# jkulhanek/wild-gaussians

Measured on AMD Instinct MI355X. Metric: train_iters_per_s (fwd+bwd of the rasterizer, 1M Gaussians @1080p), higher is better.
Workload: dtype f32

## Files before the change

wild-gaussians_amd/build.py:

```python
#!/usr/bin/env python3
from __future__ import annotations

import os
import subprocess
import sys
from concurrent.futures import ThreadPoolExecutor

HERE = os.path.dirname(os.path.abspath(__file__))
CSRC = os.path.join(HERE, "csrc")
OBJ = os.path.join(HERE, "build")
OUT = os.path.join(HERE, "diff_gaussian_rasterization", "libwg_rasterizer.so")
INCLUDE = os.path.join(os.path.dirname(HERE), "include")

VARIANT = os.environ.get("WG_BUILD_VARIANT", "")
EXTRA = os.environ.get("WG_EXTRA_FLAGS", "").split()
FILE_EXTRA = {k: v.split() for k, v in (kv.split(":", 1) for kv in filter(None, os.environ.get("WG_FILE_FLAGS", "").split(";")))}
if VARIANT:
    OBJ = os.path.join(OBJ, VARIANT)
    OUT = os.path.join(OBJ, "libwg_rasterizer.so")
HIPCC = os.environ.get("HIPCC", "/opt/rocm/bin/hipcc")
COMMON = ["--offload-arch=gfx950", "-O3", "-std=c++17", "-fPIC", "-Wall", "-Wno-unused-function", "-I" + INCLUDE, "-I" + CSRC]
SOURCES = {
    "preprocess.hip": ["-ffp-contract=off", "-fno-slp-vectorize"],
    "project/project.hip": ["-ffp-contract=off", "-fno-slp-vectorize"],
# ... 5 lines not shown
    "binning.hip": ["-fno-slp-vectorize"],
    "render_fwd.hip": ["-fno-slp-vectorize"],
    "render_bwd.hip": ["-munsafe-fp-atomics", "-fno-slp-vectorize"],
    "colour_bwd/fixed_order.hip": ["-fno-slp-vectorize"],
    "preprocess_bwd.hip": ["-fno-slp-vectorize"],
    "api.hip": [],
    "knn.hip": ["-ffp-contract=off"],
    "ssim.hip": [],
    "activations.hip": ["-ffp-contract=off"],
    "densify.hip": [],
    "sh_eval.hip": [],
    "adam.hip": ["-ffp-contract=off"],
    "adam/adam_rows.hip": ["-ffp-contract=off"],
    "appearance/mlp.hip": [],
    "appearance/colour.hip": [],
    "appearance/rows.hip": [],
    "uncertainty/uncertainty.hip": [],
    "frames/frames.hip": [],
    "metrics/metrics.hip": ["-ffp-contract=off"],
    "dino/vit.hip": [],
    "lpips/lpips.hip": ["-ffp-contract=off"],
    "loss/step_loss.hip": [],
}
HEADERS = ["wg_common.h", "wg_alpha.h", "wg_sort.h", "wg_act.h", os.path.join("distortion", "distortion.h"), os.path.join(INCLUDE, "wg_rasterizer.h"), os.path.join(INCLUDE, "wg_knn.h"),
           os.path.join(INCLUDE, "wg_ssim.h"), os.path.join(INCLUDE, "wg_activations.h"), os.path.join(INCLUDE, "wg_densify.h"), os.path.join(INCLUDE, "wg_adam.h"), os.path.join(INCLUDE, "wg_adam_rows.h"), os.path.join(INCLUDE, "wg_sh_eval.h"),
           os.path.join(INCLUDE, "wg_filter3d.h"), os.path.join(INCLUDE, "wg_densify_prune.h"), os.path.join(INCLUDE, "wg_msssim.h"),
           os.path.join(INCLUDE, "wg_appearance_mlp.h"), os.path.join(INCLUDE, "wg_appearance_colour.h"),
           os.path.join(INCLUDE, "wg_appearance_rows.h"),
           os.path.join(INCLUDE, "wg_uncertainty.h"), os.path.join(INCLUDE, "wg_frames.h"),
           os.path.join(INCLUDE, "wg_metrics.h"), os.path.join(INCLUDE, "wg_dino.h"), os.path.join(INCLUDE, "wg_lpips.h"),
           os.path.join(INCLUDE, "wg_step_loss.h")]


def _newer(target: str, deps) -> bool:
    if not os.path.exists(target):
        return True
    t = os.path.getmtime(target)
    return any(os.path.getmtime(d) > t for d in deps)


def build(force: bool = False, verbose: bool = False) -> str:
    os.makedirs(OBJ, exist_ok=True)
    hdrs = [h if os.path.isabs(h) else os.path.join(CSRC, h) for h in HEADERS] + [os.path.abspath(__file__)]
    jobs = []
    objs = []
    for src, extra in SOURCES.items():
        s = os.path.join(CSRC, src)
# ... 92 lines not shown
```

wild-gaussians_amd/csrc/api.hip:

```cpp
#include "wg_common.h"
#include "distortion/distortion.h"

#include <dlfcn.h>
#include <limits>

#include <algorithm>
#include <atomic>
#include <chrono>
#include <cstdio>
#include <cstdlib>
#include <cstring>
#include <map>
#include <mutex>
#include <string>
#include <vector>

namespace {

thread_local std::string g_last_hip_error;

int hip_fail(hipError_t e, const char* where) {
    g_last_hip_error = std::string(where) + ": " + hipGetErrorString(e);
    return WG_ERR_HIP;
}
// ... 510 lines not shown
        g_order_tables.push_back({dev, nullptr, 0});
        return nullptr;
    }
    g_order_tables.push_back({dev, static_cast<uint32_t*>(p), slots});
    *slots_out = slots;
    return static_cast<uint32_t*>(p);
}
void order_tables_release() {
    std::lock_guard<std::mutex> l(g_order_mu);
    for (OrderTable& t : g_order_tables)
        if (t.mem) {
            int cur = 0;
            const bool sw = hipGetDevice(&cur) == hipSuccess && cur != t.dev && hipSetDevice(t.dev) == hipSuccess;
            (void)hipFree(t.mem);
            if (sw) (void)hipSetDevice(cur);
        }
    g_order_tables.clear();
}

struct FrameMode { const void* image; int exact; int row; const void* geom; size_t clean_floats; };
std::atomic<uint64_t> g_row_frames{0}, g_row_backwards{0};
std::atomic<uint64_t> g_clean_frames{0}, g_clean_backwards{0};
std::atomic<uint64_t> g_sh_skip_backwards{0};
std::atomic<uint64_t> g_contribution_calls{0};
std::atomic<uint64_t> g_depth_grad_backwards{0};
std::atomic<uint64_t> g_distortion_calls{0}, g_distortion_grad_backwards{0};
std::mutex g_mode_mu;
FrameMode g_modes[64];
unsigned g_mode_head = 0;
const void* image_key(const char* image_buffer) {
    return reinterpret_cast<const void*>((reinterpret_cast<uintptr_t>(image_buffer) + wg::ALIGN - 1) & ~(uintptr_t)(wg::ALIGN - 1));
}
void remember_mode(const char* image_buffer, int exact, int row, const char* geom_buffer, size_t clean_floats) {
    const void* k = image_key(image_buffer);
    const void* gk = image_key(geom_buffer);
    std::lock_guard<std::mutex> l(g_mode_mu);
    for (auto& m : g_modes)
        if (m.image == k) { m.exact = exact; m.row = row; m.geom = gk; m.clean_floats = clean_floats; return; }
    g_modes[g_mode_head++ % 64] = {k, exact, row, gk, clean_floats};
}
bool take_record_clean(const char* image_buffer, const char* geom_buffer, size_t floats) {
    const void* k = image_key(image_buffer);
    const void* gk = image_key(geom_buffer);
    std::lock_guard<std::mutex> l(g_mode_mu);
    for (auto& m : g_modes)
        if (m.image == k) {
// ... 522 lines not shown
#endif
        if (e != hipSuccess) return hip_fail(e, "deterministic backward scratch");
    }
    const size_t record_floats = (size_t)P * (wg::GRAD_REC_FLOATS + (dual ? 1 : 0));
    bool record_clean = take_record_clean(a.image_buffer, a.geom_buffer, record_floats) && record && !det && R > 0;
    if (record_clean) {
        hipStreamCaptureStatus capturing = hipStreamCaptureStatusNone;
        if (hipStreamIsCapturing(stream, &capturing) != hipSuccess) { (void)hipGetLastError(); record_clean = false; }
        else if (capturing != hipStreamCaptureStatusNone) record_clean = false;
    }
    if (record_clean) g_clean_backwards.fetch_add(1, std::memory_order_relaxed);
    const bool clear_records = record && !det && !record_clean;
    if (clear_records && R <= 0) {
        StageScope scope_(WG_STAGE_RENDER_BACKWARD, stream);
        hipError_t e = hipMemsetAsync(geom.grad_rec, 0, (size_t)P * (wg::GRAD_REC_FLOATS + (dual ? 1 : 0)) * sizeof(float), stream);
        if (e != hipSuccess) return hip_fail(e, "gradient record memset");
    }
    const bool sh_fill = WG_SH_GRAD_SKIP != 0 && R > 0 && shs != nullptr && dL_dsh != nullptr && tone == nullptr && tone2 == nullptr && !sh_second && !dual;
    const bool nt_stream = opt.sh_stream == 1 || (opt.sh_stream < 0 && P <= opt.sh_stream_max_p);
    if (sh_fill) g_sh_skip_backwards.fetch_add(1, std::memory_order_relaxed);
    if (R > 0) {
        float* const clear_ptr = det ? reinterpret_cast<float*>(det_flags) : (clear_records ? geom.grad_rec : nullptr);
        const size_t clear_floats = det ? ((size_t)R + 3) / 4 : (size_t)P * (wg::GRAD_REC_FLOATS + (dual ? 1 : 0));
        WG_STAGE(WG_STAGE_TILE_RANGES, wg::launch_tile_order(img.tile_last, nullptr, img.order_bwd, gx * gy, clear_ptr, clear_floats, opt.backward_order_period, stream), "tile_order");
        WG_STAGE(WG_STAGE_RENDER_BACKWARD, wg::launch_render_backward(width, height, gx, gy, img, bin, geom, subpixel_offset, background, dL_dpix,
                                            dL_dmean2D, dL_dconic, dL_dopacity, dL_dcolor, record, opt.exact_compositing != 0, dual ? second->dL_dpix2 : nullptr, det_slots, det_flags, (size_t)R, P, stream,
                                            sh_fill ? dL_dsh : nullptr, sh_fill ? (size_t)P * (size_t)M * 3 : 0, WG_SH_GRAD_FILL_NT != 0 && nt_stream),
                 "render_backward");
    }
    if (dgrad != nullptr) {
        {
            StageScope scope_(WG_STAGE_RENDER_DEPTH_BACKWARD, stream);
            hipError_t e = hipMemsetAsync(dgrad->dL_dvalues, 0, (size_t)P * sizeof(float), stream);
            if (e != hipSuccess) return hip_fail(e, "dL_dvalues memset");
        }
        if (R > 0) {
            g_depth_grad_backwards.fetch_add(1, std::memory_order_relaxed);
            WG_STAGE(WG_STAGE_RENDER_DEPTH_BACKWARD, wg::launch_render_depth_backward(width, height, gx, gy, img, bin, geom, subpixel_offset, dgrad->dL_ddepth,
                                                                                    dgrad->values, means3D, campos, dgrad->dL_dvalues,
                                                                                    opt.exact_compositing != 0, stream), "render_depth_backward");
        }
    }
    if (tgrad != nullptr) {
        {
            StageScope scope_(WG_STAGE_RENDER_DEPTH_BACKWARD, stream);
            hipError_t e = hipMemsetAsync(tgrad->dL_dvalues, 0, (size_t)P * sizeof(float), stream);
            if (e != hipSuccess) return hip_fail(e, "distortion dL_dvalues memset");
        }
        if (R > 0) {
            g_distortion_grad_backwards.fetch_add(1, std::memory_order_relaxed);
// ... 301 lines not shown
    out->order_key = img.order_key;
    out->order_bwd = img.order_bwd;
    return WG_OK;
}

enum class OptKind { Flag, Tri, Range, ClampLow, ZeroOneOr };
struct OptionRow {
    const char* name;
    int (*get)(const wg::Options&);
    void (*set)(wg::Options&, int);
    OptKind kind; int lo, hi;
    void (*after_set)();
};
#define WG_OPTION(name, member, ...) {name, [](const wg::Options& o) { return (int)o.member; }, [](wg::Options& o, int v) { o.member = static_cast<decltype(o.member)>(v); }, __VA_ARGS__}
static const OptionRow g_option_rows[] = {
    WG_OPTION("force_global_sort", force_global_sort, OptKind::Flag, 0, 0, nullptr),
    WG_OPTION("host_mailbox", use_mailbox, OptKind::Flag, 0, 0, nullptr),
    WG_OPTION("geometry_reuse", geometry_reuse, OptKind::Flag, 0, 0, nullptr),
    WG_OPTION("fused_scan", fused_scan, OptKind::Flag, 0, 0, nullptr),
    WG_OPTION("forward_order", forward_order, OptKind::Flag, 0, 0, nullptr),
    WG_OPTION("forward_order_slots", forward_order_slots, OptKind::Range, 0, 1 << 16, nullptr),
    WG_OPTION("order_period", order_period, OptKind::Range, 0, 4096, nullptr),
    WG_OPTION("backward_order_period", backward_order_period, OptKind::Range, 0, 4096, nullptr),
    WG_OPTION("lazy_colour", lazy_colour, OptKind::Flag, 0, 0, nullptr),
    WG_OPTION("lazy_colour_min_p", lazy_colour_min_p, OptKind::Range, 0, 0x7fffffff, nullptr),
    WG_OPTION("sh_stream", sh_stream, OptKind::Tri, 0, 0, nullptr),
    WG_OPTION("sh_stream_max_p", sh_stream_max_p, OptKind::Range, 0, 0x7fffffff, nullptr),
    WG_OPTION("speculative_forward", speculative, OptKind::Range, 0, 2, [] { t_spec.clear(); t_wait.clear(); t_deferred.pending = false; }),
    WG_OPTION("spec_margin_pct", spec_margin_pct, OptKind::Range, 0, 1000, nullptr),
    WG_OPTION("band_list_min_p", band_list_min_p, OptKind::ClampLow, 1, 0, nullptr),
    WG_OPTION("near_split", near_split, OptKind::Tri, 0, 0, [] { t_split.reset(true); }),
    WG_OPTION("near_per_tile", near_per_tile, OptKind::ClampLow, 0, 0, nullptr),
    WG_OPTION("near_adapt", near_adapt, OptKind::Flag, 0, 0, [] { t_split.reset(false); }),
    WG_OPTION("box_count", box_count, OptKind::Tri, 0, 0, nullptr),
    WG_OPTION("depth_codes", depth_codes, OptKind::ZeroOneOr, 8, 12, nullptr),
    WG_OPTION("staged_scatter", staged_scatter, OptKind::Tri, 0, 0, nullptr),
    WG_OPTION("staged_scatter_cap", staged_cap, OptKind::ClampLow, 0, 0, nullptr),
    WG_OPTION("lazy_sort", lazy.enabled, OptKind::Flag, 0, 0, nullptr),
    WG_OPTION("lazy_min_len", lazy.min_len, OptKind::Range, 256, 2048, nullptr),
    WG_OPTION("lazy_target", lazy.target, OptKind::Range, 1, 2048, nullptr),
    WG_OPTION("lazy_cap", lazy.cap, OptKind::Range, 1, 2048, nullptr),
};
#undef WG_OPTION
static const OptionRow* find_option(const char* name) {
    for (const OptionRow& r : g_option_rows)
        if (std::strcmp(name, r.name) == 0) return &r;
// ... 25 lines not shown
    r->set(g_opt, value);
    if (r->after_set) r->after_set();
    return WG_OK;
}

int wg_get_option(const char* name) {
    if (!name) return -1;
    if (std::strcmp(name, "roctx") == 0) return g_roctx.enabled ? 1 : 0;
    if (std::strcmp(name, "near_split_backoff") == 0) return (int)t_split.backoff;
    if (std::strcmp(name, "near_per_tile_now") == 0) return (int)t_split.near.cur;
    if (std::strcmp(name, "near_floor_now") == 0) return (int)t_split.near.floor;
    if (std::strcmp(name, "near_far_tiles_last") == 0) return (int)t_split.near.last_far;
    if (std::strcmp(name, "spec_frames") == 0) return (int)std::min<uint64_t>(t_wait.spec_frames, 0x7fffffffu);
    if (std::strcmp(name, "spec_misses") == 0) return (int)std::min<uint64_t>(t_wait.spec_misses, 0x7fffffffu);
    if (std::strcmp(name, "forward_polls") == 0) return (int)std::min<uint64_t>(t_wait.polls, 0x7fffffffu);
    if (std::strcmp(name, "forward_polls_waited") == 0) return (int)std::min<uint64_t>(t_wait.waited, 0x7fffffffu);
    if (std::strcmp(name, "forward_wait_us_total") == 0) return (int)std::min(t_wait.wait_us, 2147483647.0);
    if (std::strcmp(name, "forward_wait_us_last") == 0) return (int)std::min(t_wait.last_wait_us, 2147483647.0);
    if (std::strcmp(name, "backward_row_frames") == 0) return (int)std::min<uint64_t>(g_row_frames.load(std::memory_order_relaxed), 0x7fffffffu);
    if (std::strcmp(name, "backward_row_calls") == 0) return (int)std::min<uint64_t>(g_row_backwards.load(std::memory_order_relaxed), 0x7fffffffu);
    if (std::strcmp(name, "record_clean_frames") == 0) return (int)std::min<uint64_t>(g_clean_frames.load(std::memory_order_relaxed), 0x7fffffffu);
    if (std::strcmp(name, "record_clean_calls") == 0) return (int)std::min<uint64_t>(g_clean_backwards.load(std::memory_order_relaxed), 0x7fffffffu);
    if (std::strcmp(name, "sh_grad_skip_calls") == 0) return (int)std::min<uint64_t>(g_sh_skip_backwards.load(std::memory_order_relaxed), 0x7fffffffu);
    if (std::strcmp(name, "depth_grad_calls") == 0) return (int)std::min<uint64_t>(g_depth_grad_backwards.load(std::memory_order_relaxed), 0x7fffffffu);
    if (std::strcmp(name, "distortion_calls") == 0) return (int)std::min<uint64_t>(g_distortion_calls.load(std::memory_order_relaxed), 0x7fffffffu);
    if (std::strcmp(name, "distortion_grad_calls") == 0) return (int)std::min<uint64_t>(g_distortion_grad_backwards.load(std::memory_order_relaxed), 0x7fffffffu);
    if (std::strcmp(name, "contribution_calls") == 0) return (int)std::min<uint64_t>(g_contribution_calls.load(std::memory_order_relaxed), 0x7fffffffu);
    const OptionRow* r = find_option(name);
    return r ? r->get(options_snapshot()) : -1;
}

int wg_profile_enable(int enable) {
    g_prof.enabled = enable != 0;
    return WG_OK;
}

int wg_profile_reset(void) {
    std::lock_guard<std::mutex> l(g_prof.mu);
    for (auto& r : g_prof.pending) { g_prof.pool[r.dev].push_back(r.a); g_prof.pool[r.dev].push_back(r.b); }
    g_prof.pending.clear();
    g_prof.totals = wg_stage_times{};
    return WG_OK;
}

int wg_profile_read(wg_stage_times* out) {
    if (!out) return WG_ERR_INVALID_ARGUMENT;
// ... 43 lines not shown
```

wild-gaussians_amd/csrc/binning.hip:

```cpp
#include <algorithm>
#include <cstring>
#include <cstdlib>
#include <map>
#include <mutex>
#include <utility>
#include "wg_common.h"
#include "wg_sort.h"

#include <rocprim/rocprim.hpp>

namespace wg {

uint32_t higher_msb(uint32_t n) { return n <= 1u ? 1u : 32u - (uint32_t)__builtin_clz(n); }

size_t query_scan_temp_bytes(size_t P) {
    size_t bytes = 0;
    (void)rocprim::inclusive_scan(nullptr, bytes, (uint32_t*)nullptr, (uint32_t*)nullptr, P ? P : 1, rocprim::plus<uint32_t>());
    return bytes;
}

size_t query_sort_temp_bytes(size_t R) {
    size_t bytes = 0;
    (void)rocprim::radix_sort_pairs(nullptr, bytes, (uint64_t*)nullptr, (uint64_t*)nullptr, (uint32_t*)nullptr, (uint32_t*)nullptr,
                                    R ? R : 1, 0, 64);
    return bytes;
}

bool GeometryState::band_lists_possible(size_t P) { return (P + BIN_CHUNKS - 1) / BIN_CHUNKS <= 65535; }

GeometryState GeometryState::fromChunk(char*& chunk, size_t P, bool lists, bool rows) {
// ... 421 lines not shown
        stats->split_active = active;
        const uint32_t fail = (spec.capacity != 0u && (total > spec.capacity || gmax > spec.max_list)) ? 1u : 0u;
        stats->spec_fail = fail;
        if (mailbox) {
            const unsigned long long hi = (unsigned long long)seq << 32;
            __hip_atomic_store(&mailbox->word0, hi | total, __ATOMIC_RELAXED, __HIP_MEMORY_SCOPE_SYSTEM);
            __hip_atomic_store(&mailbox->word1, hi | ((unsigned long long)fail << 31) | ((unsigned long long)active << 30) | min(gmax, MAILBOX_MAX_LIST),
                               __ATOMIC_RELAXED, __HIP_MEMORY_SCOPE_SYSTEM);
        }
    }
#pragma unroll
    for (int k = 0; k < PER; k++) {
        const int t = seg0 + 64 * k + lane;
        if (k < per && t < tiles) {
            const uint32_t c = tile_count[t], run = wave_base + cnt[k];
            tile_offset[t] = run;
            ranges[t] = c ? make_uint2(run, run + c) : make_uint2(0u, 0u);
        }
    }
}

template <typename CostFn>
__device__ __forceinline__ void order_band(CostFn cost_of, uint32_t start, uint32_t cnt, uint32_t* __restrict__ order, uint32_t period,
                                           uint32_t* hist, uint32_t* wmax) {
    const uint32_t tid = threadIdx.x, lane = tid & 63, wave = tid >> 6;
    uint32_t m = 0;
    for (uint32_t i = tid; i < cnt; i += 1024) m = max(m, cost_of(i));
#pragma unroll
    for (int d = 32; d >= 1; d >>= 1) m = max(m, (uint32_t)__shfl_xor((int)m, d));
    if (lane == 0) wmax[wave] = m;
    if (tid < 256) hist[tid] = 0;
    __syncthreads();
    m = 0;
    for (int w = 0; w < 16; w++) m = max(m, wmax[w]);
    const float scale = 255.0f / (float)max(m, 1u);
    auto bin_of = [&](uint32_t c) { return 255u - min(255u, (uint32_t)((float)c * scale)); };
    for (uint32_t i = tid; i < cnt; i += 1024) atomicAdd(&hist[bin_of(cost_of(i))], 1u);
    __syncthreads();
    if (tid < 64) {
        uint32_t v[4], sum = 0;
#pragma unroll
        for (int k = 0; k < 4; k++) { v[k] = hist[4 * tid + k]; sum += v[k]; }
        uint32_t incl = sum;
#pragma unroll
        for (int d = 1; d < 64; d <<= 1) {
            const uint32_t up = (uint32_t)__shfl_up((int)incl, d);
            if (lane >= (uint32_t)d) incl += up;
        }
        uint32_t run = incl - sum;
#pragma unroll
        for (int k = 0; k < 4; k++) { hist[4 * tid + k] = run; run += v[k]; }
    }
    __syncthreads();
    for (uint32_t i = tid; i < cnt; i += 1024) {
        uint32_t rank = atomicAdd(&hist[bin_of(cost_of(i))], 1u);
        if (period != 0u) {
            const uint32_t r = rank / period, j = rank - r * period;
            const uint32_t len = min(period, cnt - r * period);
            rank = r * period + ((r & 1u) ? len - 1u - j : j);
        }
        order[start + rank] = start + i;
    }
}

__device__ __forceinline__ void forward_order_body(int band, const FwdOrderArgs& a, int tiles, uint32_t* hist, uint32_t* wmax, uint32_t* s_key) {
    if (threadIdx.x == 0) {
        unsigned long long h = 0xcbf29ce484222325ull;
        auto mix = [&](uint32_t w) { h = (h ^ (unsigned long long)w) * 0x100000001b3ull; };
        for (int i = 0; i < 16; i++) mix(__float_as_uint(a.viewmatrix[i]));
        for (int i = 0; i < 16; i++) mix(__float_as_uint(a.projmatrix[i]));
        mix((uint32_t)a.W); mix((uint32_t)a.H);
        h ^= h >> 29;
        const uint32_t per = ((uint32_t)tiles + a.stride - 1u) / a.stride;
        const uint32_t groups = a.slots / per;
        const uint32_t slot = (uint32_t)(h % (unsigned long long)groups) * per;
        const uint32_t lo = (uint32_t)h, hi = (uint32_t)(h >> 32) | 1u;
        const uint32_t* tag = a.table + 2 * (size_t)slot;
        s_key[0] = slot; s_key[1] = lo; s_key[2] = hi;
        s_key[3] = (tag[0] == lo && tag[1] == hi) ? 1u : 0u;
        if (band == 0) { a.key_out[0] = slot; a.key_out[1] = lo; a.key_out[2] = hi; a.key_out[3] = s_key[3]; }
    }
    __syncthreads();
    const int q = tiles >> 3, rem = tiles & 7, x = band;
    const uint32_t start = x * q + min(x, rem), cnt = q + (x < rem ? 1 : 0);
// ... 486 lines not shown
    const uint32_t begin = tile_offset[tile];
    const uint32_t n = tile_near ? tile_near[tile] : tile_offset[tile + 1] - begin;
    if (n == 0) {
        if (threadIdx.x == 0) seg_end[tile] = 0;
        return;
    }
    const uint32_t* src = bucket_ids + begin;
    uint32_t len = n;
    if (n > min_len) {
        len = extract_front(bucket_ids + begin, n, depths, 0ull, n, target, cap, id_mask, sc);
        src = sc.ids;
    }
    if (len <= 512) tile_sort_body<2>(skeys, len, src, depths, point_list + begin, id_mask);
    else if (len <= 1024) tile_sort_body<4>(skeys, len, src, depths, point_list + begin, id_mask);
    else tile_sort_body<8>(skeys, len, src, depths, point_list + begin, id_mask);
    if (threadIdx.x == 0) seg_end[tile] = len;
}

__global__ void __launch_bounds__(1024) tile_order_kernel(const uint32_t* __restrict__ cost, const uint2* __restrict__ ranges,
                                                          uint32_t* __restrict__ order, int tiles, float4* __restrict__ clear, size_t clear_vec4,
                                                          uint32_t period) {
    __shared__ uint32_t hist[256];
    __shared__ uint32_t wmax[16];
    if (blockIdx.x >= 8) {
        const size_t stride = (size_t)(gridDim.x - 8) * 1024;
        for (size_t i = (size_t)(blockIdx.x - 8) * 1024 + threadIdx.x; i < clear_vec4; i += stride) clear[i] = make_float4(0.f, 0.f, 0.f, 0.f);
        return;
    }
    const int q = tiles >> 3, rem = tiles & 7, x = blockIdx.x;
    const uint32_t start = x * q + min(x, rem), cnt = q + (x < rem ? 1 : 0);
    order_band([&](uint32_t i) { return cost ? cost[start + i] : (ranges[start + i].y - ranges[start + i].x); }, start, cnt, order, period, hist, wmax);
}

hipError_t launch_tile_order(const uint32_t* cost_or_null, const uint2* ranges_or_null, uint32_t* order, int tiles, float* clear, size_t clear_floats,
                             int period, hipStream_t stream) {
    if (tiles <= 0) return hipSuccess;
    const size_t vec4 = clear ? (clear_floats + 3) / 4 : 0;
    const unsigned clear_blocks = vec4 ? (unsigned)std::min<size_t>(2048, (vec4 + 4095) / 4096) : 0u;
    hipLaunchKernelGGL(tile_order_kernel, dim3(8 + clear_blocks), dim3(1024), 0, stream, cost_or_null, ranges_or_null, order, tiles,
                       reinterpret_cast<float4*>(clear), vec4, (uint32_t)std::max(period, 0));
    return hipGetLastError();
}

static hipError_t ensure_lds(const void* fn, size_t bytes) {
    if (bytes <= 64 * 1024) return hipSuccess;
    static std::mutex mu;
    static std::map<std::pair<int, const void*>, size_t> granted;
    int dev = 0;
    hipError_t e = hipGetDevice(&dev);
    if (e != hipSuccess) return e;
    std::lock_guard<std::mutex> lock(mu);
    size_t& have = granted[{dev, fn}];
    if (bytes <= have) return hipSuccess;
    e = hipFuncSetAttribute(fn, hipFuncAttributeMaxDynamicSharedMemorySize, (int)bytes);
// ... 130 lines not shown
```

wild-gaussians_amd/csrc/render_bwd.hip:

```cpp
#include <algorithm>
#include "wg_common.h"
#include "wg_alpha.h"

namespace wg {

constexpr int BATCH = 64;

#ifndef WG_COUNT_PAIRS
#define WG_COUNT_PAIRS 0
#endif
#if WG_COUNT_PAIRS
__device__ unsigned long long g_bwd_counters[16];
#define WG_CNT(i, v) wgc[i] += (unsigned long long)(v)
#else
#define WG_CNT(i, v)
#endif

typedef float f2 __attribute__((ext_vector_type(2)));

template <int CTRL>
__device__ __forceinline__ float dpp_f(float v) {
    return __builtin_bit_cast(float, __builtin_amdgcn_update_dpp(0, __builtin_bit_cast(int, v), CTRL, 0xF, 0xF, false));
}

__device__ __forceinline__ float pair_x32(float a, float b) {
// ... 80 lines not shown
    const size_t stop = begin + per_wave < nvec ? begin + per_wave : nvec;
    const float4 z = make_float4(0.f, 0.f, 0.f, 0.f);
    if (nt) { for (size_t i = begin + threadIdx.x; i < stop; i += 64) stream_store4<true>(&body[i], z); }
    else { for (size_t i = begin + threadIdx.x; i < stop; i += 64) body[i] = z; }
    if (blockIdx.x == 0) {
        const size_t tail = head + 4 * nvec;
        if (threadIdx.x < head) fill[threadIdx.x] = 0.f;
        if (tail + threadIdx.x < n) fill[tail + threadIdx.x] = 0.f;
    }
}
template <bool RECORD, bool DET = false, bool EXACT = false, bool DUAL = false>
__global__ void __launch_bounds__(64) WG_BWD_OCC
#if WG_BWD_DUAL_WAVES
__attribute__((amdgpu_waves_per_eu(DUAL ? WG_BWD_DUAL_WAVES : 1, DUAL ? WG_BWD_DUAL_WAVES : 8)))
#endif
render_backward_kernel(
    int W, int H, int gx, int tiles, const uint32_t* __restrict__ order, const uint2* __restrict__ ranges, const uint32_t* __restrict__ point_list,
    const float4* __restrict__ splats, const float2* __restrict__ subpixel_offset, const float* __restrict__ bg,
    const float* __restrict__ final_T, const uint32_t* __restrict__ n_contrib, const uint32_t* __restrict__ tile_last,
    const float* __restrict__ dL_dpix, float* __restrict__ dL_dmean2D, float* __restrict__ dL_dconic,
    float* __restrict__ dL_dopacity, float* __restrict__ dL_dcolor, float* __restrict__ grad_rec,
    const ushort4* __restrict__ rects, const uint32_t* __restrict__ offsets_incl, const uint32_t* __restrict__ tiles_touched,
    float* __restrict__ det_slots, unsigned char* __restrict__ det_flags, const float* __restrict__ dL_dpix2, float* __restrict__ grad_aux,
    float* __restrict__ fill, size_t fill_floats, uint32_t fill_per_wave, int fill_nt) {
    static_assert(!DUAL || RECORD, "the two-colour walk accumulates into the gradient record (or, DET, into fourteen-float slots)");
    constexpr int SLOT_FLOATS = DUAL ? 14 : 10;
    constexpr int RS = DUAL ? 4 : 3;
    constexpr bool LDSRED = WG_BWD_LDS_REDUCE != 0;
    constexpr int NS = DUAL ? 7 : 5;
    __shared__ float4 smem[(LDSRED ? 16 * NS : 0) + BATCH * RS];
    float4* const lds = smem + (LDSRED ? 16 * NS : 0);
    float* const red = reinterpret_cast<float*>(smem);

#if WG_PROBE
    const unsigned long long probe_t0 = __builtin_amdgcn_s_memrealtime();
#endif
    const int tile = (int)order[xcd_tile(blockIdx.x, tiles)];
    const int hi0 = (int)tile_last[tile];
#if WG_PROBE
    if (hi0 == 0 && threadIdx.x == 0 && blockIdx.x < 65536) {
        g_bwd_probe[4 * blockIdx.x] = probe_t0; g_bwd_probe[4 * blockIdx.x + 1] = probe_t0; g_bwd_probe[4 * blockIdx.x + 3] = (unsigned long long)tile;
        g_bwd_probe[4 * blockIdx.x + 2] = ((unsigned long long)__builtin_amdgcn_s_getreg((20 << 0) | (0 << 6) | (31 << 11)) << 32) | (unsigned)__builtin_amdgcn_s_getreg((4 << 0) | (0 << 6) | (31 << 11));
    }
#endif
    if (hi0 == 0) {
        bwd_fill_zero(fill, fill_floats, fill_per_wave, fill_nt);
        return;
    }
    const int lane = threadIdx.x;
    const int tx = tile % gx, ty = tile / gx;
    const size_t plane = (size_t)W * H;
    const float bg0 = bg[0], bg1 = bg[1], bg2 = bg[2];
    const float ddelx_dx = 0.5f * W, ddely_dy = 0.5f * H;

    const int red_m = (lane & 31) >> 2, red_half = lane >> 5;
    const int vidx = LDSRED ? min(2 * red_m + red_half, DUAL ? 12 : 9)
                   : DUAL ? 8 * ((lane >> 1) & 1) + 4 * (lane & 1) + 2 * ((lane >> 4) & 1) + ((lane >> 5) & 1)
                          : ((lane & 2) ? 8 + ((lane >> 5) & 1) : 4 * (lane & 1) + 2 * ((lane >> 4) & 1) + ((lane >> 5) & 1));
    const bool owner = (lane & 12) == 0;
    float* abase;
// ... 351 lines not shown
            if (c == 0u) continue;
            if (nb + c > 64u) { reduce_batch(nb); nb = 0u; }
            if (flagged[u]) batch[nb + (uint32_t)__popcll(m & ((1ull << lane) - 1ull))] = glo + 64u * u + (uint32_t)lane;
            nb += c;
        }
    }
    if (nb != 0u) reduce_batch(nb);
    if (valid) {
        float4* out = reinterpret_cast<float4*>(grad_rec + (size_t)g * GRAD_REC_FLOATS);
        out[0] = make_float4(acc[0], acc[1], acc[2], acc[3]);
        out[1] = make_float4(acc[4], acc[5], acc[6], acc[7]);
        if (NF2 == 5) out[2] = make_float4(acc[8], acc[9], 0.f, 0.f);
        else {
            out[2] = make_float4(acc[8], acc[9], acc[NF2 == 5 ? 0 : 10], acc[NF2 == 5 ? 0 : 11]);
            grad_rec[(size_t)P * GRAD_REC_FLOATS + g] = acc[NF2 == 5 ? 0 : 12];
        }
    }
}

hipError_t launch_render_backward(int W, int H, int gx, int gy, const ImageState& img, const BinningState& b,
                                  const GeometryState& g, const float* subpixel_offset, const float* background,
                                  const float* dL_dpix, float* dL_dmean2D, float* dL_dconic, float* dL_dopacity,
                                  float* dL_dcolor, bool record, bool exact, const float* dL_dpix2, float* det_slots, unsigned char* det_flags, size_t slot_capacity, int P,
                                  hipStream_t stream, float* fill, size_t fill_floats, bool fill_nt) {
    const int tiles = gx * gy;
    if (tiles <= 0) return hipSuccess;
    const uint32_t fill_per_wave = fill ? (uint32_t)((fill_floats / 4 + (size_t)tiles - 1) / (size_t)tiles) : 0u;
#define WG_LAUNCH3(REC, DET, EX, DU)                                                                                                            \
    hipLaunchKernelGGL((render_backward_kernel<REC, DET, EX, DU>), dim3(tiles), dim3(64), 0, stream, W, H, gx, tiles, img.order_bwd, img.ranges,     \
                       b.point_list, g.splats, reinterpret_cast<const float2*>(subpixel_offset), background, img.final_T, img.n_contrib,    \
                       img.tile_last, dL_dpix, dL_dmean2D, dL_dconic, dL_dopacity, dL_dcolor, g.grad_rec, g.rects, g.point_offsets,         \
                       g.tiles_touched, det_slots, det_flags, dL_dpix2, g.grad_rec + (size_t)P * GRAD_REC_FLOATS, fill, fill_floats, fill_per_wave,    \
                       fill_nt ? 1 : 0)
#define WG_LAUNCH2(REC, DET, EX) WG_LAUNCH3(REC, DET, EX, false)
#define WG_LAUNCH(REC, DET) do { if (exact) WG_LAUNCH2(REC, DET, true); else WG_LAUNCH2(REC, DET, false); } while (0)
    if (dL_dpix2 && det_slots) {
        if (exact) WG_LAUNCH3(true, true, true, true); else WG_LAUNCH3(true, true, false, true);
        hipLaunchKernelGGL(det_reduce_kernel<7>, dim3((P + 255) / 256), dim3(256), 0, stream, P, g.point_offsets, g.tiles_touched, det_slots, det_flags,
                           g.grad_rec, slot_capacity);
    } else if (dL_dpix2) {
        if (exact) WG_LAUNCH3(true, false, true, true); else WG_LAUNCH3(true, false, false, true);
    } else if (det_slots) {
        WG_LAUNCH(true, true);
        hipLaunchKernelGGL(det_reduce_kernel<5>, dim3((P + 255) / 256), dim3(256), 0, stream, P, g.point_offsets, g.tiles_touched, det_slots, det_flags,
                           g.grad_rec, slot_capacity);
    } else if (record) WG_LAUNCH(true, false);
    else WG_LAUNCH(false, false);
#undef WG_LAUNCH
#undef WG_LAUNCH2
#undef WG_LAUNCH3
    return hipGetLastError();
}

template <bool EXACT>
__global__ void __launch_bounds__(64) render_backward_colour_kernel(
    int W, int H, int gx, int tiles, const uint32_t* __restrict__ order, const uint2* __restrict__ ranges, const uint32_t* __restrict__ point_list,
// ... 158 lines not shown
```

wild-gaussians_amd/csrc/wg_common.h:

```cpp
#pragma once
#include <hip/hip_runtime.h>
#include <stdint.h>
#include <stddef.h>
#include <type_traits>
#include "../../include/wg_rasterizer.h"

namespace wg {

constexpr int TILE_X = WG_TILE_X;
constexpr int TILE_Y = WG_TILE_Y;
constexpr size_t ALIGN = 256;

template <typename T>
__host__ inline void carve(char*& chunk, T*& ptr, size_t count) {
    uintptr_t p = (reinterpret_cast<uintptr_t>(chunk) + ALIGN - 1) & ~(uintptr_t)(ALIGN - 1);
    ptr = reinterpret_cast<T*>(p);
    chunk = reinterpret_cast<char*>(ptr + count);
}

struct GeometryState {
    float* depths;
    int* radii;
    float4* splats;
    float* cov3D;
// ... 294 lines not shown
struct Options {
    LazyConfig lazy;
    int staged_scatter = -1;
    int staged_cap = 0;
    int band_list_min_p = 2000000;
    int depth_codes = 1;
    int speculative = 1;
    int spec_margin_pct = 25;
    int fused_scan = 0;
    int geometry_reuse = 0;
    int exact_compositing = 1;
    int grad_record = 1;
    int deterministic_backward = 0;
    int near_split = -1;
    int near_per_tile = 0;
    int near_adapt = 1;
    int box_count = -1;
    bool force_global_sort = false;
    bool use_mailbox = true;
    int forward_order = 1;
    int forward_order_slots = 2048;
    int order_period = 128;
    int backward_order_period = 0;
    int lazy_colour = 1;
    int lazy_colour_min_p = 4000000;
    int sh_stream = -1;
    int sh_stream_max_p = 6000000;
};
hipError_t launch_tile_sort_lazy(const ImageState& img, const BinningState& b, const GeometryState& g, int tiles, int code_bits,
                                 const LazyConfig& lazy, bool split, const BinStats* guard, hipStream_t stream);
hipError_t launch_render_fixup(int code_bits, int W, int H, int gx, int gy, const ImageState& img, const BinningState& b, const GeometryState& g,
                               const float* subpixel_offset, const float* background, float* out_color, float* out_color2, const LazyConfig& lazy,
                               bool split, int phase, bool exact, HostMailbox* mailbox_dev, const BinStats* guard, hipStream_t stream);
hipError_t launch_tile_sort(const ImageState& img, const BinningState& b, const GeometryState& g, int tiles, uint32_t max_count,
                            const BinStats* guard, hipStream_t stream);
hipError_t launch_render_forward(int W, int H, int gx, int gy, const ImageState& img, const BinningState& b,
                                 const GeometryState& g, const float* subpixel_offset, const float* background,
                                 float* out_color, float* out_color2, bool lazy, bool exact, const BinStats* guard, float* record_clear,
                                 size_t record_floats, uint32_t* order_table,
                                 uint32_t order_slots, uint32_t order_stride, hipStream_t stream);
hipError_t launch_poison_unfit(const ImageState& img, int W, int H, int tiles, float* out_color, float* out_color2, hipStream_t stream);
hipError_t launch_render_forward_replay(int W, int H, int gx, int gy, const ImageState& img, const BinningState& b,
                                        const GeometryState& g, const float* subpixel_offset, const float* background,
                                        float* out_color, bool exact, hipStream_t stream);
hipError_t launch_render_backward(int W, int H, int gx, int gy, const ImageState& img, const BinningState& b,
                                  const GeometryState& g, const float* subpixel_offset, const float* background,
                                  const float* dL_dpix, float* dL_dmean2D, float* dL_dconic, float* dL_dopacity,
                                  float* dL_dcolor, bool record, bool exact, const float* dL_dpix2, float* det_slots, unsigned char* det_flags, size_t slot_capacity, int P,
                                  hipStream_t stream, float* fill = nullptr, size_t fill_floats = 0, bool fill_nt = false);
#ifndef WG_SH_GRAD_SKIP
#define WG_SH_GRAD_SKIP 1
#endif
#ifndef WG_SH_GRAD_FILL_NT
#define WG_SH_GRAD_FILL_NT 1
#endif
hipError_t launch_render_backward_colour(int W, int H, int gx, int gy, const ImageState& img, const BinningState& b, const GeometryState& g,
                                         const float* subpixel_offset, const float* dL_dpix, float* dL_dcolor, bool exact, hipStream_t stream);
hipError_t launch_render_backward_colour_fixed(int W, int H, int gx, int gy, const ImageState& img, const BinningState& b, const GeometryState& g,
                                               const float* subpixel_offset, const float* dL_dpix, float* dL_dcolor, bool exact, float* slots,
                                               unsigned char* flags, size_t slot_capacity, int P, hipStream_t stream);
hipError_t launch_render_depth(int W, int H, int gx, int gy, const ImageState& img, const BinningState& b, const GeometryState& g,
                               const float* subpixel_offset, const float* values, const float* means3D, const float* campos, float* depth,
                               bool exact, hipStream_t stream);
hipError_t launch_render_depth_backward(int W, int H, int gx, int gy, const ImageState& img, const BinningState& b, const GeometryState& g,
                                        const float* subpixel_offset, const float* dL_ddepth, const float* values, const float* means3D,
                                        const float* campos, float* dL_dvalues, bool exact, hipStream_t stream);
hipError_t launch_depth_distance_fold(int P, const float* means3D, const float* campos, const float* dL_dvalues, float* dL_dmean3D, hipStream_t stream);
hipError_t launch_render_contrib(int W, int H, int gx, int gy, const ImageState& img, const BinningState& b, const GeometryState& g,
                                 const float* subpixel_offset, const float* pixel_mask, float* max_weight, unsigned long long* hits,
                                 unsigned long long* weight_sum_q32, bool exact, hipStream_t stream);

struct BwdParams {
// ... 28 lines not shown
```

Before: 1100.

## Let backward render blocks select their own tile order instead of a separate launch

Adds a default-on option that skips the tile_order kernel in the backward pass when gradient records are already clean. Instead, each render_backward block runs a wave-level histogram select over its XCD band's tile costs and finds the tile it should process. It also writes that choice to order_bwd for later use. The shared order_band routine is also changed to rank tiles with a ballot-based stable placement, so the standalone kernel and the in-kernel selector produce the same order. This removes one launch and a dependency point, but every block now re-reads about a thousand band costs and does histogram and select work before it starts rendering.

After: 1095. No clear change (-0.5%).

```diff
diff --git a/wild-gaussians_amd/build.py b/wild-gaussians_amd/build.py
--- a/wild-gaussians_amd/build.py
+++ b/wild-gaussians_amd/build.py
@@ -51,7 +51,7 @@
     "lpips/lpips.hip": ["-ffp-contract=off"],
     "loss/step_loss.hip": [],
 }
-HEADERS = ["wg_common.h", "wg_alpha.h", "wg_sort.h", "wg_act.h", os.path.join("distortion", "distortion.h"), os.path.join(INCLUDE, "wg_rasterizer.h"), os.path.join(INCLUDE, "wg_knn.h"),
+HEADERS = ["wg_common.h", "wg_alpha.h", "wg_sort.h", "wg_act.h", os.path.join("order", "wg_order.h"), os.path.join("distortion", "distortion.h"), os.path.join(INCLUDE, "wg_rasterizer.h"), os.path.join(INCLUDE, "wg_knn.h"),
            os.path.join(INCLUDE, "wg_ssim.h"), os.path.join(INCLUDE, "wg_activations.h"), os.path.join(INCLUDE, "wg_densify.h"), os.path.join(INCLUDE, "wg_adam.h"), os.path.join(INCLUDE, "wg_adam_rows.h"), os.path.join(INCLUDE, "wg_sh_eval.h"),
            os.path.join(INCLUDE, "wg_filter3d.h"), os.path.join(INCLUDE, "wg_densify_prune.h"), os.path.join(INCLUDE, "wg_msssim.h"),
            os.path.join(INCLUDE, "wg_appearance_mlp.h"), os.path.join(INCLUDE, "wg_appearance_colour.h"),
diff --git a/wild-gaussians_amd/csrc/api.hip b/wild-gaussians_amd/csrc/api.hip
--- a/wild-gaussians_amd/csrc/api.hip
+++ b/wild-gaussians_amd/csrc/api.hip
@@ -556,6 +556,7 @@
 std::atomic<uint64_t> g_row_frames{0}, g_row_backwards{0};
 std::atomic<uint64_t> g_clean_frames{0}, g_clean_backwards{0};
 std::atomic<uint64_t> g_sh_skip_backwards{0};
+std::atomic<uint64_t> g_self_order_backwards{0};
 std::atomic<uint64_t> g_contribution_calls{0};
 std::atomic<uint64_t> g_depth_grad_backwards{0};
 std::atomic<uint64_t> g_distortion_calls{0}, g_distortion_grad_backwards{0};
@@ -1124,10 +1125,13 @@
     if (R > 0) {
         float* const clear_ptr = det ? reinterpret_cast<float*>(det_flags) : (clear_records ? geom.grad_rec : nullptr);
         const size_t clear_floats = det ? ((size_t)R + 3) / 4 : (size_t)P * (wg::GRAD_REC_FLOATS + (dual ? 1 : 0));
-        WG_STAGE(WG_STAGE_TILE_RANGES, wg::launch_tile_order(img.tile_last, nullptr, img.order_bwd, gx * gy, clear_ptr, clear_floats, opt.backward_order_period, stream), "tile_order");
+        const bool self_order = opt.backward_self_order != 0 && record_clean;
+        if (self_order) g_self_order_backwards.fetch_add(1, std::memory_order_relaxed);
+        else WG_STAGE(WG_STAGE_TILE_RANGES, wg::launch_tile_order(img.tile_last, nullptr, img.order_bwd, gx * gy, clear_ptr, clear_floats, opt.backward_order_period, stream), "tile_order");
         WG_STAGE(WG_STAGE_RENDER_BACKWARD, wg::launch_render_backward(width, height, gx, gy, img, bin, geom, subpixel_offset, background, dL_dpix,
                                             dL_dmean2D, dL_dconic, dL_dopacity, dL_dcolor, record, opt.exact_compositing != 0, dual ? second->dL_dpix2 : nullptr, det_slots, det_flags, (size_t)R, P, stream,
-                                            sh_fill ? dL_dsh : nullptr, sh_fill ? (size_t)P * (size_t)M * 3 : 0, WG_SH_GRAD_FILL_NT != 0 && nt_stream),
+                                            sh_fill ? dL_dsh : nullptr, sh_fill ? (size_t)P * (size_t)M * 3 : 0, WG_SH_GRAD_FILL_NT != 0 && nt_stream,
+                                            self_order ? opt.backward_order_period : -1),
                  "render_backward");
     }
     if (dgrad != nullptr) {
@@ -1475,6 +1479,7 @@
     WG_OPTION("forward_order_slots", forward_order_slots, OptKind::Range, 0, 1 << 16, nullptr),
     WG_OPTION("order_period", order_period, OptKind::Range, 0, 4096, nullptr),
     WG_OPTION("backward_order_period", backward_order_period, OptKind::Range, 0, 4096, nullptr),
+    WG_OPTION("backward_self_order", backward_self_order, OptKind::Flag, 0, 0, nullptr),
     WG_OPTION("lazy_colour", lazy_colour, OptKind::Flag, 0, 0, nullptr),
     WG_OPTION("lazy_colour_min_p", lazy_colour_min_p, OptKind::Range, 0, 0x7fffffff, nullptr),
     WG_OPTION("sh_stream", sh_stream, OptKind::Tri, 0, 0, nullptr),
@@ -1546,6 +1551,7 @@
     if (std::strcmp(name, "record_clean_frames") == 0) return (int)std::min<uint64_t>(g_clean_frames.load(std::memory_order_relaxed), 0x7fffffffu);
     if (std::strcmp(name, "record_clean_calls") == 0) return (int)std::min<uint64_t>(g_clean_backwards.load(std::memory_order_relaxed), 0x7fffffffu);
     if (std::strcmp(name, "sh_grad_skip_calls") == 0) return (int)std::min<uint64_t>(g_sh_skip_backwards.load(std::memory_order_relaxed), 0x7fffffffu);
+    if (std::strcmp(name, "backward_self_order_calls") == 0) return (int)std::min<uint64_t>(g_self_order_backwards.load(std::memory_order_relaxed), 0x7fffffffu);
     if (std::strcmp(name, "depth_grad_calls") == 0) return (int)std::min<uint64_t>(g_depth_grad_backwards.load(std::memory_order_relaxed), 0x7fffffffu);
     if (std::strcmp(name, "distortion_calls") == 0) return (int)std::min<uint64_t>(g_distortion_calls.load(std::memory_order_relaxed), 0x7fffffffu);
     if (std::strcmp(name, "distortion_grad_calls") == 0) return (int)std::min<uint64_t>(g_distortion_grad_backwards.load(std::memory_order_relaxed), 0x7fffffffu);
diff --git a/wild-gaussians_amd/csrc/binning.hip b/wild-gaussians_amd/csrc/binning.hip
--- a/wild-gaussians_amd/csrc/binning.hip
+++ b/wild-gaussians_amd/csrc/binning.hip
@@ -6,6 +6,7 @@
 #include <utility>
 #include "wg_common.h"
 #include "wg_sort.h"
+#include "order/wg_order.h"
 
 #include <rocprim/rocprim.hpp>
 
@@ -473,7 +474,7 @@
 
 template <typename CostFn>
 __device__ __forceinline__ void order_band(CostFn cost_of, uint32_t start, uint32_t cnt, uint32_t* __restrict__ order, uint32_t period,
-                                           uint32_t* hist, uint32_t* wmax) {
+                                           uint32_t* hist, uint32_t* wmax, uint32_t* whist = nullptr) {
     const uint32_t tid = threadIdx.x, lane = tid & 63, wave = tid >> 6;
     uint32_t m = 0;
     for (uint32_t i = tid; i < cnt; i += 1024) m = max(m, cost_of(i));
@@ -484,8 +485,8 @@
     __syncthreads();
     m = 0;
     for (int w = 0; w < 16; w++) m = max(m, wmax[w]);
-    const float scale = 255.0f / (float)max(m, 1u);
-    auto bin_of = [&](uint32_t c) { return 255u - min(255u, (uint32_t)((float)c * scale)); };
+    const float scale = order_scale(m);
+    auto bin_of = [&](uint32_t c) { return order_bin(c, scale); };
     for (uint32_t i = tid; i < cnt; i += 1024) atomicAdd(&hist[bin_of(cost_of(i))], 1u);
     __syncthreads();
     if (tid < 64) {
@@ -503,14 +504,42 @@
         for (int k = 0; k < 4; k++) { hist[4 * tid + k] = run; run += v[k]; }
     }
     __syncthreads();
-    for (uint32_t i = tid; i < cnt; i += 1024) {
-        uint32_t rank = atomicAdd(&hist[bin_of(cost_of(i))], 1u);
-        if (period != 0u) {
-            const uint32_t r = rank / period, j = rank - r * period;
-            const uint32_t len = min(period, cnt - r * period);
-            rank = r * period + ((r & 1u) ? len - 1u - j : j);
-        }
-        order[start + rank] = start + i;
+    if (whist == nullptr) {
+        for (uint32_t i = tid; i < cnt; i += 1024) {
+            const uint32_t rank = atomicAdd(&hist[bin_of(cost_of(i))], 1u);
+            order[start + order_snake(rank, period, cnt)] = start + i;
+        }
+        return;
+    }
+    for (uint32_t i0 = 0; i0 < cnt; i0 += 1024) {
+        for (uint32_t k = tid; k < 16 * 256; k += 1024) whist[k] = 0;
+        __syncthreads();
+        const uint32_t i = i0 + tid;
+        const bool valid = i < cnt;
+        const uint32_t b = valid ? bin_of(cost_of(i)) : 0xffffffffu;
+        uint32_t place = 0;
+        uint64_t todo = __ballot(valid);
+        while (todo != 0ull) {
+            const int l = __builtin_ctzll(todo);
+            const uint32_t bb = (uint32_t)__shfl((int)b, l);
+            const uint64_t same = __ballot(b == bb);
+            if (b == bb) place = (uint32_t)__popcll(same & ((1ull << lane) - 1ull));
+            if (lane == (uint32_t)l) whist[256 * wave + bb] = (uint32_t)__popcll(same);
+            todo &= ~same;
+        }
+        __syncthreads();
+        if (tid < 256) {
+            uint32_t run = hist[tid];
+            for (int w = 0; w < 16; w++) {
+                const uint32_t v = whist[256 * w + tid];
+                whist[256 * w + tid] = run;
+                run += v;
+            }
+            hist[tid] = run;
+        }
+        __syncthreads();
+        if (valid) order[start + order_snake(whist[256 * wave + b] + place, period, cnt)] = start + i;
+        __syncthreads();
     }
 }
 
@@ -1043,6 +1072,7 @@
                                                           uint32_t period) {
     __shared__ uint32_t hist[256];
     __shared__ uint32_t wmax[16];
+    __shared__ uint32_t whist[16 * 256];
     if (blockIdx.x >= 8) {
         const size_t stride = (size_t)(gridDim.x - 8) * 1024;
         for (size_t i = (size_t)(blockIdx.x - 8) * 1024 + threadIdx.x; i < clear_vec4; i += stride) clear[i] = make_float4(0.f, 0.f, 0.f, 0.f);
@@ -1050,7 +1080,7 @@
     }
     const int q = tiles >> 3, rem = tiles & 7, x = blockIdx.x;
     const uint32_t start = x * q + min(x, rem), cnt = q + (x < rem ? 1 : 0);
-    order_band([&](uint32_t i) { return cost ? cost[start + i] : (ranges[start + i].y - ranges[start + i].x); }, start, cnt, order, period, hist, wmax);
+    order_band([&](uint32_t i) { return cost ? cost[start + i] : (ranges[start + i].y - ranges[start + i].x); }, start, cnt, order, period, hist, wmax, whist);
 }
 
 hipError_t launch_tile_order(const uint32_t* cost_or_null, const uint2* ranges_or_null, uint32_t* order, int tiles, float* clear, size_t clear_floats,
diff --git a/wild-gaussians_amd/csrc/order/wg_order.h b/wild-gaussians_amd/csrc/order/wg_order.h
--- /dev/null
+++ b/wild-gaussians_amd/csrc/order/wg_order.h
@@ -0,0 +1,125 @@
+#pragma once
+#include <stdint.h>
+
+#if defined(__HIPCC__) || defined(__CUDACC__)
+#define WG_ORDER_HD __host__ __device__ __forceinline__
+#else
+#define WG_ORDER_HD inline
+#endif
+
+namespace wg {
+
+WG_ORDER_HD float order_scale(uint32_t max_cost) { return 255.0f / (float)(max_cost > 1u ? max_cost : 1u); }
+WG_ORDER_HD uint32_t order_bin(uint32_t cost, float scale) {
+    const uint32_t v = (uint32_t)((float)cost * scale);
+    return 255u - (v < 255u ? v : 255u);
+}
+WG_ORDER_HD uint32_t order_snake(uint32_t rank, uint32_t period, uint32_t cnt) {
+    if (period == 0u) return rank;
+    const uint32_t r = rank / period, j = rank - r * period;
+    const uint32_t left = cnt - r * period, len = period < left ? period : left;
+    return r * period + ((r & 1u) ? len - 1u - j : j);
+}
+
+WG_ORDER_HD uint32_t order_select_serial(const uint32_t* cost, uint32_t cnt, uint32_t slot, uint32_t period) {
+    if (slot >= cnt) return cnt;
+    uint32_t m = 0;
+    for (uint32_t i = 0; i < cnt; i++) m = cost[i] > m ? cost[i] : m;
+    const float scale = order_scale(m);
+    uint32_t hist[256];
+    for (uint32_t b = 0; b < 256u; b++) hist[b] = 0u;
+    for (uint32_t i = 0; i < cnt; i++) hist[order_bin(cost[i], scale)]++;
+    uint32_t rank = order_snake(slot, period, cnt), bin = 0u;
+    while (rank >= hist[bin]) rank -= hist[bin++];
+    for (uint32_t i = 0; i < cnt; i++)
+        if (order_bin(cost[i], scale) == bin && rank-- == 0u) return i;
+    return cnt;
+}
+
+#if defined(__HIPCC__)
+template <int CTRL, int ROWS>
+__device__ __forceinline__ uint32_t order_dpp_max(uint32_t v) {
+    const uint32_t o = (uint32_t)__builtin_amdgcn_update_dpp((int)v, (int)v, CTRL, ROWS, 0xF, false);
+    return o > v ? o : v;
+}
+
+__device__ __forceinline__ uint32_t order_select_wave(const uint32_t* __restrict__ cost, uint32_t cnt, uint32_t slot, uint32_t period,
+                                                      uint32_t* hist) {
+    constexpr int PER = 16;
+    const uint32_t lane = threadIdx.x & 63u;
+    const bool one = cnt <= 64u * PER;
+    uint32_t c[PER];
+    auto load_round = [&](uint32_t base) {
+#pragma unroll
+        for (int k = 0; k < PER; k++) {
+            const uint32_t i = base + 64u * k + lane;
+            c[k] = i < cnt ? cost[i] : 0u;
+        }
+    };
+    load_round(0u);
+    uint32_t m = 0;
+    for (uint32_t base = 0; base < cnt; base += 64u * PER) {
+        if (base != 0u) load_round(base);
+#pragma unroll
+        for (int k = 0; k < PER; k++) m = c[k] > m ? c[k] : m;
+    }
+    m = order_dpp_max<0xB1, 0xF>(m); m = order_dpp_max<0x4E, 0xF>(m); m = order_dpp_max<0x124, 0xF>(m); m = order_dpp_max<0x128, 0xF>(m);
+    m = order_dpp_max<0x142, 0xA>(m); m = order_dpp_max<0x143, 0xC>(m);
+    const float scale = order_scale((uint32_t)__builtin_amdgcn_readlane((int)m, 63));
+
+    reinterpret_cast<uint4*>(hist)[lane] = make_uint4(0u, 0u, 0u, 0u);
+    __syncthreads();
+    for (uint32_t base = 0; base < cnt; base += 64u * PER) {
+        if (!one) load_round(base);
+#pragma unroll
+        for (int k = 0; k < PER; k++) {
+            const bool valid = base + 64u * k + lane < cnt;
+            c[k] = order_bin(c[k], scale);
+            if (valid) atomicAdd(&hist[c[k]], 1u);
+        }
+    }
+    __syncthreads();
+    const uint4 h = reinterpret_cast<const uint4*>(hist)[lane];
+    const uint32_t sum = h.x + h.y + h.z + h.w;
+    uint32_t incl = sum;
+#pragma unroll
+    for (int d = 1; d < 64; d <<= 1) {
+        const uint32_t up = (uint32_t)__shfl_up((int)incl, d);
+        if (lane >= (uint32_t)d) incl += up;
+    }
+    const uint32_t rank = order_snake(slot, period, cnt);
+    const uint64_t hit = __ballot(incl - sum <= rank && rank < incl);
+    const int src = hit != 0ull ? __builtin_ctzll(hit) : 0;
+    uint32_t run = (uint32_t)__shfl((int)(incl - sum), src);
+    const uint32_t h0 = (uint32_t)__shfl((int)h.x, src), h1 = (uint32_t)__shfl((int)h.y, src), h2 = (uint32_t)__shfl((int)h.z, src);
+    uint32_t bin = 4u * (uint32_t)src;
+    if (rank >= run + h0) { run += h0; bin++;
+        if (rank >= run + h1) { run += h1; bin++;
+            if (rank >= run + h2) { run += h2; bin++; } } }
+    uint32_t left = rank - run;
+    uint32_t found = 0u;
+    bool done = false;
+    for (uint32_t base = 0; base < cnt; base += 64u * PER) {
+        if (!one) {
+            load_round(base);
+#pragma unroll
+            for (int k = 0; k < PER; k++) c[k] = order_bin(c[k], scale);
+        }
+#pragma unroll
+        for (int k = 0; k < PER; k++) {
+            const uint64_t mask = __ballot(base + 64u * k + lane < cnt && c[k] == bin);
+            const uint32_t n = (uint32_t)__popcll(mask);
+            if (!done) {
+                if (left < n) {
+                    const uint64_t pick = __ballot(((mask >> lane) & 1ull) != 0ull && (uint32_t)__popcll(mask & ((1ull << lane) - 1ull)) == left);
+                    found = base + 64u * k + (uint32_t)__builtin_ctzll(pick);
+                    done = true;
+                } else left -= n;
+            }
+        }
+    }
+    return found;
+}
+#endif
+
+}
diff --git a/wild-gaussians_amd/csrc/render_bwd.hip b/wild-gaussians_amd/csrc/render_bwd.hip
--- a/wild-gaussians_amd/csrc/render_bwd.hip
+++ b/wild-gaussians_amd/csrc/render_bwd.hip
@@ -1,6 +1,7 @@
 #include <algorithm>
 #include "wg_common.h"
 #include "wg_alpha.h"
+#include "order/wg_order.h"
 
 namespace wg {
 
@@ -127,7 +128,7 @@
     float* __restrict__ dL_dopacity, float* __restrict__ dL_dcolor, float* __restrict__ grad_rec,
     const ushort4* __restrict__ rects, const uint32_t* __restrict__ offsets_incl, const uint32_t* __restrict__ tiles_touched,
     float* __restrict__ det_slots, unsigned char* __restrict__ det_flags, const float* __restrict__ dL_dpix2, float* __restrict__ grad_aux,
-    float* __restrict__ fill, size_t fill_floats, uint32_t fill_per_wave, int fill_nt) {
+    float* __restrict__ fill, size_t fill_floats, uint32_t fill_per_wave, int fill_nt, uint32_t* __restrict__ order_out, uint32_t order_period) {
     static_assert(!DUAL || RECORD, "the two-colour walk accumulates into the gradient record (or, DET, into fourteen-float slots)");
     constexpr int SLOT_FLOATS = DUAL ? 14 : 10;
     constexpr int RS = DUAL ? 4 : 3;
@@ -140,7 +141,16 @@
 #if WG_PROBE
     const unsigned long long probe_t0 = __builtin_amdgcn_s_memrealtime();
 #endif
-    const int tile = (int)order[xcd_tile(blockIdx.x, tiles)];
+    int tile;
+    if ((RECORD && !DET) && order_out != nullptr) {
+        const int q = tiles >> 3, rem = tiles & 7, x = (int)blockIdx.x & 7;
+        const uint32_t start = (uint32_t)(x * q + min(x, rem)), cnt = (uint32_t)(q + (x < rem ? 1 : 0));
+        const uint32_t found = order_select_wave(tile_last + start, cnt, blockIdx.x >> 3, order_period, reinterpret_cast<uint32_t*>(smem));
+        tile = __builtin_amdgcn_readfirstlane((int)(start + found));
+        if (threadIdx.x == 0) order_out[xcd_tile(blockIdx.x, tiles)] = (uint32_t)tile;
+    } else {
+        tile = (int)order[xcd_tile(blockIdx.x, tiles)];
+    }
     const int hi0 = (int)tile_last[tile];
 #if WG_PROBE
     if (hi0 == 0 && threadIdx.x == 0 && blockIdx.x < 65536) {
@@ -538,16 +548,19 @@
                                   const GeometryState& g, const float* subpixel_offset, const float* background,
                                   const float* dL_dpix, float* dL_dmean2D, float* dL_dconic, float* dL_dopacity,
                                   float* dL_dcolor, bool record, bool exact, const float* dL_dpix2, float* det_slots, unsigned char* det_flags, size_t slot_capacity, int P,
-                                  hipStream_t stream, float* fill, size_t fill_floats, bool fill_nt) {
+                                  hipStream_t stream, float* fill, size_t fill_floats, bool fill_nt, int self_order_period) {
     const int tiles = gx * gy;
     if (tiles <= 0) return hipSuccess;
     const uint32_t fill_per_wave = fill ? (uint32_t)((fill_floats / 4 + (size_t)tiles - 1) / (size_t)tiles) : 0u;
+    if (self_order_period >= 0 && (!record || det_slots)) return hipErrorInvalidValue;
+    uint32_t* const order_out = self_order_period >= 0 ? img.order_bwd : nullptr;
+    const uint32_t order_period = (uint32_t)std::max(self_order_period, 0);
 #define WG_LAUNCH3(REC, DET, EX, DU)                                                                                                            \
     hipLaunchKernelGGL((render_backward_kernel<REC, DET, EX, DU>), dim3(tiles), dim3(64), 0, stream, W, H, gx, tiles, img.order_bwd, img.ranges,     \
                        b.point_list, g.splats, reinterpret_cast<const float2*>(subpixel_offset), background, img.final_T, img.n_contrib,    \
                        img.tile_last, dL_dpix, dL_dmean2D, dL_dconic, dL_dopacity, dL_dcolor, g.grad_rec, g.rects, g.point_offsets,         \
                        g.tiles_touched, det_slots, det_flags, dL_dpix2, g.grad_rec + (size_t)P * GRAD_REC_FLOATS, fill, fill_floats, fill_per_wave,    \
-                       fill_nt ? 1 : 0)
+                       fill_nt ? 1 : 0, order_out, order_period)
 #define WG_LAUNCH2(REC, DET, EX) WG_LAUNCH3(REC, DET, EX, false)
 #define WG_LAUNCH(REC, DET) do { if (exact) WG_LAUNCH2(REC, DET, true); else WG_LAUNCH2(REC, DET, false); } while (0)
     if (dL_dpix2 && det_slots) {
diff --git a/wild-gaussians_amd/csrc/wg_common.h b/wild-gaussians_amd/csrc/wg_common.h
--- a/wild-gaussians_amd/csrc/wg_common.h
+++ b/wild-gaussians_amd/csrc/wg_common.h
@@ -340,6 +340,7 @@
     int forward_order_slots = 2048;
     int order_period = 128;
     int backward_order_period = 0;
+    int backward_self_order = 1;
     int lazy_colour = 1;
     int lazy_colour_min_p = 4000000;
     int sh_stream = -1;
@@ -365,7 +366,7 @@
                                   const GeometryState& g, const float* subpixel_offset, const float* background,
                                   const float* dL_dpix, float* dL_dmean2D, float* dL_dconic, float* dL_dopacity,
                                   float* dL_dcolor, bool record, bool exact, const float* dL_dpix2, float* det_slots, unsigned char* det_flags, size_t slot_capacity, int P,
-                                  hipStream_t stream, float* fill = nullptr, size_t fill_floats = 0, bool fill_nt = false);
+                                  hipStream_t stream, float* fill = nullptr, size_t fill_floats = 0, bool fill_nt = false, int self_order_period = -1);
 #ifndef WG_SH_GRAD_SKIP
 #define WG_SH_GRAD_SKIP 1
 #endif
```
